# mp3guy/ElasticFusion

Measured on AMD Instinct MI355X. Metric: frames/s per GPU, 640x480 3-level ICP+fuse, higher is better.
Workload: dtype f32

## Files before the change

### elasticfusion_amd/csrc/ef_map_kernels.hip

```cpp
#include "ef_device.hpp"
#include <stdlib.h>
#include <mutex>
#include <hip/hip_ext.h>
#include "ef_map.hpp"
#include "ef_zkey.hpp"

using namespace ef;

namespace efm {

namespace {

inline int ceil_div(int a, int b) { return (a + b - 1) / b; }
constexpr int SURFEL_GRID = 1024;
constexpr int BLK = 256;
constexpr int CLEAN_GRID = 4096;
static_assert(CLEAN_ROW == BLK, "clean kernels run one element per thread");
static_assert(CLEAN_GRID % 8 == 0, "xcd_row");

__device__ __forceinline__ unsigned long long zkey(float z, uint32_t id) { return ((unsigned long long)depth_key(z) << 32) | id; }
__device__ __forceinline__ unsigned xcd_block() {
  const unsigned g = gridDim.x, x = blockIdx.x & 7u, slot = blockIdx.x >> 3;
  return x * (g >> 3) + (x < (g & 7u) ? x : (g & 7u)) + slot;
}
// ... 379 lines not shown
                                                        const unsigned* __restrict__ count_dev, float maxDepth, float confThreshold,
                                                        int time, int maxTime, int timeDelta, unsigned long long* zbuf,
                                                        unsigned* consumed_mark, unsigned consumed_value, const float4* __restrict__ rays) {
  if (consumed_mark && blockIdx.x == 0 && threadIdx.x == 0)
    __hip_atomic_store(consumed_mark, consumed_value, __ATOMIC_RELAXED, __HIP_MEMORY_SCOPE_SYSTEM);
  const rt34 T = rt34_load16(T16);
  const unsigned count = *count_dev;
  const unsigned sub = threadIdx.x % SPLAT_LANES;
  const unsigned stride = gridDim.x * blockDim.x / SPLAT_LANES;
  for (unsigned id = (blockIdx.x * blockDim.x + threadIdx.x) / SPLAT_LANES; id < count; id += stride) {
    const float4 pc = map.pos_conf[id];
    if (pc.w < confThreshold) continue;
    const float4 ct = map.col_time[id];
    const float4 nr = map.nrm_rad[id];
    const Sprite S = make_sprite(cam, T, pc, ct, nr, maxDepth, confThreshold, (float)time, (float)maxTime, (float)timeDelta);
    if (!S.ok) continue;
    const int px0 = max(0, (int)ceilf(S.u - S.hs - 0.5f)), px1 = min(cam.cols - 1, (int)ceilf(S.u + S.hs - 0.5f) - 1);
    const int py0 = max(0, (int)ceilf(S.v - S.hs - 0.5f)), py1 = min(cam.rows - 1, (int)ceilf(S.v + S.hs - 0.5f) - 1);
    const int hgt = py1 - py0 + 1, nfrag = (px1 - px0 + 1) * hgt;
    const float psn = dot(S.p, S.n);
    for (int f = (int)sub; f < nfrag; f += SPLAT_LANES) {
      const int fx = f / hgt, py = py0 + (f - fx * hgt), px = px0 + fx;
      const int zi = px * cam.rows + py;
      f3 l;
      if (LUT) { const float4 r = rays[zi]; l = f3{r.x, r.y, r.z}; }
      else l = pixel_ray(cam, px, py);
      float z;
      if (!sprite_fragment_ray(S.p, S.n, S.rad, psn, l, z)) continue;
      if (z != z) continue;
      unsigned long long* cell = &zbuf[zi];
      const unsigned long long key = zkey(z, id);
      atomicMin(cell, key);
    }
  }
}

__device__ __forceinline__ f3 fill_vertex_at(const uint16_t* __restrict__ d, const Cam& cam, int sx, int sy, int x, int y, float inv_fx,
                                             float inv_fy) {
  const float z = (float)d[clampi(sy, 0, cam.rows - 1) * cam.cols + clampi(sx, 0, cam.cols - 1)] / 1000.0f;
  return {((float)x - cam.cx) * z * inv_fx, ((float)y - cam.cy) * z * inv_fy, z};
}
__device__ __forceinline__ void fill_in_px(const Cam& cam, int x, int y, uchar4 si, float4 sv, float4 sn,
                                           const uint16_t* __restrict__ depth_filtered, const uint8_t* __restrict__ rgb3, bool passthrough,
                                           bool passthroughImage, FillMaps out) {
  const int pi = y * cam.cols + x;
  const float inv_fx = 1.0f / cam.fx, inv_fy = 1.0f / cam.fy;
  if (sv.z == 0 || passthrough) {
    const f3 v = fill_vertex_at(depth_filtered, cam, x, y, x, y, inv_fx, inv_fy);
    out.vertex[pi] = make_float4(v.x, v.y, v.z, 1.f);
  } else {
    out.vertex[pi] = sv;
  }
  if (sn.z == 0 || passthrough) {
    const f3 v = fill_vertex_at(depth_filtered, cam, x, y, x, y, inv_fx, inv_fy);
    const f3 vx = fill_vertex_at(depth_filtered, cam, x + 1, y, x + 1, y, inv_fx, inv_fy);
    const f3 vy = fill_vertex_at(depth_filtered, cam, x, y + 1, x, y + 1, inv_fx, inv_fy);
    const f3 nn = normalized(cross(vx - v, vy - v));
    out.normal[pi] = make_float4(nn.x, nn.y, nn.z, 1.f);
  } else {
    out.normal[pi] = sn;
  }
  if ((si.x == 0 && si.y == 0 && si.z == 0) || passthroughImage) {
    out.image[pi] = make_uchar4(rgb3[(size_t)pi * 3], rgb3[(size_t)pi * 3 + 1], rgb3[(size_t)pi * 3 + 2], 255);
  } else {
    out.image[pi] = si;
  }
}
__device__ __forceinline__ void dense_sample(const Cam& cam, int x, int y, uchar4 si, unsigned* counter) {
  if (counter && x % 20 == 10 && y % 20 == 10 && x / 20 < cam.cols / 20 && y / 20 < cam.rows / 20)
    if (si.x > 0 && si.y > 0 && si.z > 0) atomicAdd(counter, 1u);
}

template <bool FUSE_FILL>
__global__ void __launch_bounds__(BLK) k_surface_resolve(const Cam cam, const float* __restrict__ T16, SurfelSoA map, float maxDepth,
                                                          float confThreshold, int time, int maxTime, int timeDelta,
                                                          unsigned long long* zbuf, PredictMaps out, FillMaps fill,
                                                          const uint16_t* __restrict__ depth_filtered, const uint8_t* __restrict__ rgb3,
                                                          bool passthroughImage, unsigned* dense_counter, unsigned* nonempty_flag,
                                                          unsigned nonempty_value) {
  const int lane = threadIdx.x & 63, wave = threadIdx.x >> 6;
  const int px = blockIdx.x * 16 + (wave & 1) * 8 + (lane >> 3), py = blockIdx.y * 16 + (wave >> 1) * 8 + (lane & 7);
  if (px >= cam.cols || py >= cam.rows) return;
  const int pi = py * cam.cols + px, zi = px * cam.rows + py;
  const unsigned long long key = zbuf[zi];
  uchar4 im = make_uchar4(0, 0, 0, 0);
  float4 vt = make_float4(0, 0, 0, 0), nm = make_float4(0, 0, 0, 0);
  uint16_t tm = 0;
  if (key != ZBUF_EMPTY) {
    if (nonempty_flag) *nonempty_flag = nonempty_value;
    zbuf[zi] = ZBUF_EMPTY;
    const uint32_t id = (uint32_t)key;
    const rt34 T = rt34_load16(T16);
    const float4 pc = map.pos_conf[id], ct = map.col_time[id], nr = map.nrm_rad[id];
    const Sprite S = make_sprite(cam, T, pc, ct, nr, maxDepth, confThreshold, (float)time, (float)maxTime, (float)timeDelta);
    float z = 0.f;
    sprite_fragment(cam, S, px, py, z);
    const f3 col = decodeColor(ct.x);
    im = make_uchar4((uint8_t)roundf(col.x * 255.0f), (uint8_t)roundf(col.y * 255.0f), (uint8_t)roundf(col.z * 255.0f), 255);
    const float fcx = (float)px + 0.5f, fcy = (float)py + 0.5f;
    vt = make_float4((fcx - cam.cx) * z * (1.f / cam.fx), (fcy - cam.cy) * z * (1.f / cam.fy), z, pc.w);
    nm = make_float4(S.n.x, S.n.y, S.n.z, nr.w);
    tm = (uint16_t)(unsigned)ct.z;
  }
  out.image[pi] = im;
  out.vertex[pi] = vt;
  out.normal[pi] = nm;
  out.time[pi] = tm;
  if (FUSE_FILL) {
    fill_in_px(cam, px, py, im, vt, nm, depth_filtered, rgb3, false, passthroughImage, fill);
    dense_sample(cam, px, py, im, dense_counter);
  }
}
__global__ void __launch_bounds__(BLK) k_depth_resolve(int cols, int rows, unsigned long long* zbuf, float* __restrict__ depth) {
  const int pi = blockIdx.x * blockDim.x + threadIdx.x;
  if (pi >= cols * rows) return;
  const int py = pi / cols, px = pi - py * cols, zi = px * rows + py;
  const unsigned long long key = zbuf[zi];
  float z = 0.f;
  if (key != ZBUF_EMPTY) {
    zbuf[zi] = ZBUF_EMPTY;
    z = depth_of_key((uint32_t)(key >> 32));
  }
  depth[pi] = z;
}
__global__ void __launch_bounds__(BLK) k_fill_in(const Cam cam, PredictMaps pred, const uint16_t* __restrict__ depth_filtered,
                                                  const uint8_t* __restrict__ rgb3, bool passthrough, bool passthroughImage, FillMaps out) {
  const int pi = blockIdx.x * blockDim.x + threadIdx.x;
  if (pi >= cam.cols * cam.rows) return;
  const int py = pi / cam.cols, px = pi - py * cam.cols;
  fill_in_px(cam, px, py, pred.image[pi], pred.vertex[pi], pred.normal[pi], depth_filtered, rgb3, passthrough, passthroughImage, out);
}
__global__ void k_dense_count(const Cam cam, const uchar4* __restrict__ image, unsigned* counter) {
  const int dc = cam.cols / 20, dr = cam.rows / 20;
  const int i = blockIdx.x * blockDim.x + threadIdx.x;
  if (i >= dc * dr) return;
  const int b = i / dc, a = i - b * dc;
  const uchar4 t = image[(20 * b + 10) * cam.cols + (20 * a + 10)];
  if (t.x > 0 && t.y > 0 && t.z > 0) atomicAdd(counter, 1u);
}

struct FuseArgs {
  Cam cam;
  const float* pose16;
  int time;
  const uint8_t* rgb3;
  const float* dm;
  const float* dmf;
  IndexMaps im;
  float maxDepth;
  const float* weighting;
  KeyedIndex key;
  unsigned long long* zclear;
};
template <bool KEYED>
__global__ void __launch_bounds__(BLK) k_associate(const FuseArgs A, Candidates cand, uint32_t* winner, int colwalk) {
  const Cam cam = A.cam;
  const int qc = cam.cols / 2, qr = cam.rows / 2;
  const int q = (int)(xcd_block() * blockDim.x + threadIdx.x);
  if (KEYED && A.zclear)
    for (int i = q, P = cam.cols * cam.rows, step = (int)(gridDim.x * blockDim.x); i < P; i += step) A.zclear[i] = ZBUF_EMPTY;
  if (q >= qc * qr) return;
  const int qy = colwalk ? q % qr : q / qc, qx = colwalk ? q / qr : q - (q / qc) * qc;
  const int par = A.time % 2;
  const int i = 2 * qx + par, j = 2 * qy + par;
  const int r = qx * qr + qy;
  float4 c_col = make_float4(0, 0, 0, 0);
  if (i < cam.cols && j < cam.rows) {
    const float cx = cam.cx, cy = cam.cy;
    const float inv_fx = (float)(1.0 / (double)cam.fx), inv_fy = (float)(1.0 / (double)cam.fy);
    const DepthF DR{A.dm, cam.cols, cam.rows}, DF{A.dmf, cam.cols, cam.rows};
    const float x = pix_coord(i, cam.cols), y = pix_coord(j, cam.rows);
    const float ftime = (float)A.time;
    const f3 vPosLocal = getVertexF(DR, i, j, x, y, cx, cy, inv_fx, inv_fy);
    const bool sel = ((int)x % 2 == (int)ftime % 2 && (int)y % 2 == (int)ftime % 2);
    const bool nb = !(DR.at(i - 1, j) == 0 || DR.at(i, j - 1) == 0 || DR.at(i + 1, j) == 0 || DR.at(i, j + 1) == 0);
    const float zf_c = DF.at(i, j), zf_xf = DF.at(i + 1, j), zf_xb = DF.at(i - 1, j), zf_yf = DF.at(i, j + 1), zf_yb = DF.at(i, j - 1);
    const uint8_t* c = A.rgb3 + (size_t)(j * cam.cols + i) * 3;
    const uint8_t c0 = c[0], c1 = c[1], c2 = c[2];
    const float weighting = *A.weighting;
    uint32_t idx9[3][3];
    float4 vc9[3][3], nr9[3][3];
    uint2 key9[3][3];
#pragma unroll
    for (int a = 0; a < 3; ++a) {
      const int tx = clampi(i + a - 1, 0, cam.cols - 1);
#pragma unroll
      for (int b = 0; b < 3; ++b) {
        const int ty = clampi(j + b - 1, 0, cam.rows - 1);
        const int ti = im_texel(A.im, cam, tx, ty);
        if (KEYED) {
          key9[a][b] = reinterpret_cast<const uint2*>(A.key.keys)[ti];
        } else {
          idx9[a][b] = A.im.index[ti];
          vc9[a][b] = A.im.vert_conf[ti];
          nr9[a][b] = A.im.norm_rad[ti];
        }
      }
    }
    const rt34 pose = rt34_load16(A.pose16);
    if (sel && nb && vPosLocal.z > 0 && vPosLocal.z <= A.maxDepth) {
      const f3 vPos = xform(pose, vPosLocal);
      auto vtx = [&](float z, float xx, float yy) { return f3{(xx - cx) * z * inv_fx, (yy - cy) * z * inv_fy, z}; };
      const f3 vPosition_f = vtx(zf_c, x, y);
      const f3 col{(float)c0 / 255.0f, (float)c1 / 255.0f, (float)c2 / 255.0f};
      const f3 xf = vtx(zf_xf, x + 1, y), xb = vtx(zf_xb, x - 1, y), yf = vtx(zf_yf, x, y + 1), yb = vtx(zf_yb, x, y - 1);
      const f3 del_x = half_sum(xb, vPosition_f) - half_sum(xf, vPosition_f);
      const f3 del_y = half_sum(yb, vPosition_f) - half_sum(yf, vPosition_f);
      const f3 vNormLocal = normalized(cross(del_x, del_y));
      const f3 nW = mul(pose.R, vNormLocal);
      int counter = 0;
      uint32_t best = 0;
      float bestDist = 1000;
      const float xl = (x - cx) * inv_fx, yl = (y - cy) * inv_fy;
      const float lambda = sqrtf(xl * xl + yl * yl + 1);
      const f3 ray{xl, yl, 1};
      const float lenRay = sqrtf(dot(ray, ray));
      const float lenN = sqrtf(dot(vNormLocal, vNormLocal));
      const rt34 Tcw = rt34_load16(KEYED ? A.key.T_cw16_dev : A.pose16);
      if (KEYED) {
#pragma unroll
        for (int a = 0; a < 3; ++a)
#pragma unroll
          for (int b = 0; b < 3; ++b) {
            const uint32_t id = key9[a][b].x;
            float vcz = depth_of_key(key9[a][b].y);
            asm volatile("" : "+v"(vcz));
            const bool tap = (id & key9[a][b].y) != 0xFFFFFFFFu  && id > 0U && fabsf((vcz * lambda) - (vPosLocal.z * lambda)) < 0.05f;
            idx9[a][b] = tap ? id : 0U;
          }
#pragma unroll
        for (int a = 0; a < 3; ++a)
#pragma unroll
          for (int b = 0; b < 3; ++b) {
            vc9[a][b] = A.key.map.pos_conf[idx9[a][b]];
            nr9[a][b] = A.key.map.nrm_rad[idx9[a][b]];
          }
      }
#pragma unroll
      for (int a = 0; a < 4; ++a) {
        const int a3 = a == 0 ? 0 : (a == 3 ? 2 : 1);
#pragma unroll
        for (int b = 0; b < 4; ++b) {
          const int b3 = b == 0 ? 0 : (b == 3 ? 2 : 1);
          const uint32_t current = idx9[a3][b3];
          if (current > 0U) {
            const float4 vc = KEYED ? index_texel_vert_conf(Tcw, vc9[a3][b3]) : vc9[a3][b3];
            if (fabsf((vc.z * lambda) - (vPosLocal.z * lambda)) < 0.05f) {
              const f3 cr = cross(ray, f3{vc.x, vc.y, vc.z});
              const float dist = sqrtf(dot(cr, cr)) / lenRay;
              const float4 nr = KEYED ? index_texel_norm_rad(Tcw, nr9[a3][b3]) : nr9[a3][b3];
              const f3 nn{nr.x, nr.y, nr.z};
              const float cang = dot(nn, vNormLocal) / (sqrtf(dot(nn, nn)) * lenN);
              const bool angOk = (cang > 0.87758255f && cang <= 1.0f);
              if (dist < bestDist && (fabsf(nr.z) < 0.75f || angOk)) {
                counter++;
                bestDist = dist;
                best = current;
              }
            }
          }
        }
      }
      const float tag = counter > 0 ? -1.0f : -2.0f;
      cand.pos_conf[r] = make_float4(vPos.x, vPos.y, vPos.z, confidence(x, y, cx, cy, weighting));
      cand.nrm_rad[r] = make_float4(nW.x, nW.y, nW.z, getRadius(vPosition_f.z, vNormLocal.z, inv_fx, inv_fy));
      c_col = make_float4(encodeColor(col), 0.f, ftime, tag);
      cand.best[r] = best;
      if (counter > 0) atomicMin(&winner[best], (uint32_t)r);
    }
  }
  cand.col_time[r] = c_col;
}
__device__ __forceinline__ void merge_surfel(const Candidates& cand, int r, uint32_t id, const SurfelSoA& map, int time, float4& s, float4& sc) {
  const float4 ucol = cand.col_time[r];
  const float4 u = cand.pos_conf[r], un = cand.nrm_rad[r];
  float4 sn = map.nrm_rad[id];
  const float c_k = s.w, a = u.w, ftime = (float)time;
  if (un.w < (1.0f + 0.5f) * sn.w) {
    s.x = ((c_k * s.x) + (a * u.x)) / (c_k + a);
    s.y = ((c_k * s.y) + (a * u.y)) / (c_k + a);
    s.z = ((c_k * s.z) + (a * u.z)) / (c_k + a);
    s.w = c_k + a;
    const f3 oldCol = decodeColor(sc.x), newCol = decodeColor(ucol.x);
    const f3 avg{((c_k * oldCol.x) + (a * newCol.x)) / (c_k + a), ((c_k * oldCol.y) + (a * newCol.y)) / (c_k + a),
                 ((c_k * oldCol.z) + (a * newCol.z)) / (c_k + a)};
    sc.x = encodeColor(avg);
    sc.w = ftime;
    const float nx = ((c_k * sn.x) + (a * un.x)) / (c_k + a), ny = ((c_k * sn.y) + (a * un.y)) / (c_k + a),
                nz = ((c_k * sn.z) + (a * un.z)) / (c_k + a), nw = ((c_k * sn.w) + (a * un.w)) / (c_k + a);
    const f3 nn = normalized(f3{nx, ny, nz});
    sn = make_float4(nn.x, nn.y, nn.z, nw);
    map.pos_conf[id] = s;
    map.col_time[id] = sc;
    map.nrm_rad[id] = sn;
  } else {
    s.w = c_k + a;
    sc.w = ftime;
    map.pos_conf[id] = s;
    map.col_time[id] = sc;
  }
}
__global__ void __launch_bounds__(BLK) k_merge(Candidates cand, const uint32_t* __restrict__ winner, SurfelSoA map, int time) {
  const int r = blockIdx.x * blockDim.x + threadIdx.x;
  if (r >= cand.n) return;
  if (cand.col_time[r].w != -1.0f) return;
  const uint32_t id = cand.best[r];
  if (winner[id] != (uint32_t)r) return;
  float4 s = map.pos_conf[id], sc = map.col_time[id];
  merge_surfel(cand, r, id, map, time, s, sc);
}

struct CleanArgs {
  Cam cam;
  const float* T16;
  int time;
  IndexMaps im;
  float confThreshold;
  int timeDelta;
  KeyedIndex key;
};
struct Taps3 { int u[3]; int m[3]; };
__device__ __forceinline__ Taps3 dedupe_taps(float x, int hi) {
  int t[4];
#pragma unroll
  for (int a = 0; a < 4; ++a) t[a] = clampi((int)floorf(x + (-1.0f + 0.5f * a)), 0, hi);
  Taps3 r;
  r.u[0] = t[0];
  r.u[2] = t[3];
  r.u[1] = (t[1] != t[0] && t[1] != t[3]) ? t[1] : t[2];
  r.m[0] = 1 + (t[1] == t[0]) + (t[2] == t[0]) + (t[3] == t[0]);
  r.m[2] = (t[3] != t[0]) ? (1 + (t[0] == t[3]) + (t[1] == t[3]) + (t[2] == t[3])) : 0;
  r.m[1] = (r.u[1] != t[0] && r.u[1] != t[3]) ? ((t[1] == r.u[1]) + (t[2] == r.u[1])) : 0;
  return r;
}
template <bool KEYED>
__device__ __forceinline__ bool clean_test(const CleanArgs& A, const rt34& T, float4 pc, float4 ct, float4 nr) {
  const Cam& cam = A.cam;
  const float ftime = (float)A.time, ftd = (float)A.timeDelta;
  int test = 1;
  const f3 localPos = xform(T, f3{pc.x, pc.y, pc.z});
  const float x = ((cam.fx * localPos.x) / localPos.z) + cam.cx;
  const float y = ((cam.fy * localPos.y) / localPos.z) + cam.cy;
  const f3 localNorm = normalized(mul(T.R, f3{nr.x, nr.y, nr.z}));
  int cnt = 0, zCount = 0;
  const float tagTime = ct.w == -2 ? ftime : ct.w;
  const bool decided = tagTime == -1 || ((ftime - tagTime) > 20 && pc.w < A.confThreshold);
  if (!decided && ftime - ct.w < ftd && localPos.z > 0 && x > 0 && y > 0 && x < (float)cam.cols && y < (float)cam.rows) {
    const Taps3 tx = dedupe_taps(x, cam.cols - 1), ty = dedupe_taps(y, cam.rows - 1);
    uint32_t idx[9];
    float4 vcs[9], c2s[9];
    if (KEYED) {
      unsigned long long keys[9];
#pragma unroll
      for (int a = 0; a < 3; ++a)
#pragma unroll
        for (int b = 0; b < 3; ++b) keys[a * 3 + b] = A.key.keys[im_texel(A.im, cam, tx.u[a], ty.u[b])];
#pragma unroll
      for (int a = 0; a < 3; ++a)
#pragma unroll
        for (int b = 0; b < 3; ++b) {
          const unsigned long long key = keys[a * 3 + b];
          const uint32_t id = (uint32_t)key;
          const bool tap = tx.m[a] * ty.m[b] > 0 && key != ZBUF_EMPTY && id > 0U && depth_of_key((uint32_t)(key >> 32)) > localPos.z;
          idx[a * 3 + b] = tap ? id : 0U;
        }
#pragma unroll
      for (int k = 0; k < 9; ++k) {
        vcs[k] = A.key.map.pos_conf[idx[k]];
        c2s[k] = A.key.map.col_time[idx[k]];
      }
    } else {
#pragma unroll
      for (int a = 0; a < 3; ++a)
#pragma unroll
        for (int b = 0; b < 3; ++b) {
          const int ti = im_texel(A.im, cam, tx.u[a], ty.u[b]);
          idx[a * 3 + b] = A.im.index[ti];
          vcs[a * 3 + b] = A.im.vert_conf[ti];
          c2s[a * 3 + b] = A.im.color_time[ti];
        }
    }
    const bool steep = fabsf(localNorm.z) > 0.85f;
#pragma unroll
    for (int a = 0; a < 3; ++a)
#pragma unroll
      for (int b = 0; b < 3; ++b) {
        const int w = tx.m[a] * ty.m[b];
        const float4 vc = KEYED ? index_texel_vert_conf(T, vcs[a * 3 + b]) : vcs[a * 3 + b], c2 = c2s[a * 3 + b];
        if (w > 0 && idx[a * 3 + b] > 0U) {
          const float dx = vc.x - localPos.x, dy = vc.y - localPos.y;
          if (c2.z < ct.z && vc.w > A.confThreshold && vc.z > localPos.z && vc.z - localPos.z < 0.01f &&
              sqrtf(dx * dx + dy * dy) < nr.w * 1.4f)
            cnt += w;
          if (c2.w == ftime && vc.w > A.confThreshold && vc.z > localPos.z && vc.z - localPos.z > 0.01f && steep)
            zCount += w;
        }
      }
  }
  if (cnt > 8 || zCount > 4) test = 0;
  float lastTime = ct.w;
  if (lastTime == -2) lastTime = ftime;
  if (lastTime == -1 || ((ftime - lastTime) > 20 && pc.w < A.confThreshold)) test = 0;
  if (lastTime > 0 && ftime - lastTime > ftd) test = 1;
  return test != 0;
}
__device__ __forceinline__ bool load_element(const SurfelSoA& map, const Candidates& cand, unsigned count, unsigned e, float4& pc,
                                             float4& ct, float4& nr) {
  if (e < count) {
    pc = map.pos_conf[e]; ct = map.col_time[e]; nr = map.nrm_rad[e];
    return true;
  }
  const unsigned r = e - count;
  ct = cand.col_time[r];
  if (ct.w == 0.0f) return false;
  pc = cand.pos_conf[r]; nr = cand.nrm_rad[r];
  return true;
}
struct DeformArgs {
  const float* graph;
  int nodes;
  const float* depth;
  int isFern;
  float maxDepth;
};
// ... 263 lines not shown
    }
    base += tot;
    __syncthreads();
  }
}

}

static inline dim3 tgrid(int cols, int rows) { return dim3(ceil_div(cols, 64), ceil_div(rows, 4)); }

const float* bilateral_table() {
  static std::mutex mu;
  static float* tables[64] = {};
  int dev = 0;
  if (hipGetDevice(&dev) != hipSuccess || dev < 0 || dev >= 64) return nullptr;
  std::lock_guard<std::mutex> lk(mu);
  if (!tables[dev]) {
    float* p = nullptr;
    if (hipMalloc(&p, sizeof(float) * BIL_ROWS * BIL_COLS) != hipSuccess) return nullptr;
    hipLaunchKernelGGL(k_bilateral_table, dim3(ceil_div(BIL_ROWS * BIL_COLS, 256)), dim3(256), 0, (hipStream_t)0, p);
    if (hipDeviceSynchronize() != hipSuccess) { (void)hipFree(p); return nullptr; }
    tables[dev] = p;
  }
  return tables[dev];
}
bool filter_depth(const uint16_t* raw, int cols, int rows, float maxD, uint16_t* filtered, hipStream_t s) {
  const float* table = bilateral_table();
  if (!table) return false;
  hipLaunchKernelGGL(k_preprocess<false>, dim3(ceil_div(cols, PRE_TW), ceil_div(rows, PRE_TH)), dim3(64, 4), 0, s, raw, cols, rows, (unsigned)(maxD * 1000.0f), table,
                     filtered, (float*)nullptr, (float*)nullptr, (const uint8_t*)nullptr, (uint8_t*)nullptr, (uint8_t*)nullptr);
  return true;
}
void metricise_depth(const uint16_t* in, int cols, int rows, float maxD, float* out, hipStream_t s) {
  hipLaunchKernelGGL(k_metricise, dim3(ceil_div(cols * rows, 256)), dim3(256), 0, s, in, cols * rows, (unsigned)(maxD * 1000.0f), out);
}
bool preprocess_depth(const uint16_t* raw, int cols, int rows, float maxD, uint16_t* filtered, float* metric, float* metric_filtered,
                      hipStream_t s, unsigned extra_lds, const uint8_t* rgb3, uint8_t* next0, uint8_t* rgb_keep, const float* table) {
  if (!table) table = bilateral_table();
  if (!table) return false;
  constexpr unsigned STATIC_LDS = sizeof(float) * (BIL_ROWS * BIL_COLS + PRE_LH * PRE_LW);
  static_assert(STATIC_LDS < 65536u, "k_preprocess fits the default LDS limit");
  if (extra_lds > 65536u - STATIC_LDS) extra_lds = 65536u - STATIC_LDS;
  hipLaunchKernelGGL(k_preprocess<true>, dim3(ceil_div(cols, PRE_TW), ceil_div(rows, PRE_TH)), dim3(64, 4), extra_lds, s, raw, cols, rows, (unsigned)(maxD * 1000.0f), table,
                     filtered, metric, metric_filtered, rgb3, next0, rgb_keep);
  return true;
}
namespace {
__global__ void k_copy_map(SurfelSoA src, const unsigned* __restrict__ count_dev, SurfelSoA dst) {
  const unsigned n = *count_dev;
  for (unsigned i = blockIdx.x * blockDim.x + threadIdx.x; i < n; i += gridDim.x * blockDim.x) {
    dst.pos_conf[i] = src.pos_conf[i];
    dst.col_time[i] = src.col_time[i];
    dst.nrm_rad[i] = src.nrm_rad[i];
  }
}
}
void copy_map(SurfelSoA src, const unsigned* count_dev, SurfelSoA dst, hipStream_t s) {
  hipLaunchKernelGGL(k_copy_map, dim3(SURFEL_GRID), dim3(BLK), 0, s, src, count_dev, dst);
}
void aos_to_soa(const float* aos, uint32_t count, SurfelSoA soa, hipStream_t s) {
  if (count) hipLaunchKernelGGL(k_aos_to_soa, dim3(ceil_div((int)count, 256)), dim3(256), 0, s, (const float4*)aos, count, soa);
}
void soa_to_aos(SurfelSoA soa, uint32_t count, float* aos, hipStream_t s) {
  if (count) hipLaunchKernelGGL(k_soa_to_aos, dim3(ceil_div((int)count, 256)), dim3(256), 0, s, soa, count, (float4*)aos);
}

void seed_map(const Cam& cam, const uint8_t* rgb3, const float* dm, const float* dmf, int time, float maxDepth, SurfelSoA out,
              unsigned* count_dev, const CompactScratch& cs, hipStream_t s) {
  const int P = cam.cols * cam.rows;
  const int nch = ceil_div(P, CHUNK);
  SeedArgs A{cam, rgb3, dm, dmf, time, maxDepth};
  uint8_t* fr = cs.flags;
  uint8_t* ff = cs.flags + P;
  uint32_t* cr = cs.chunk_count;
  uint32_t* cf = cs.chunk_count + nch;
  uint32_t* orw = cs.chunk_offset;
  uint32_t* ofl = cs.chunk_offset + nch;
  (void)hipMemsetAsync(out.nrm_rad, 0, (size_t)P * sizeof(float4), s);
  hipLaunchKernelGGL(k_seed_flags, dim3(nch), dim3(BLK), 0, s, A, fr, ff, cr, cf);
  hipLaunchKernelGGL(k_scan_chunks, dim3(1), dim3(1024), 0, s, (const uint32_t*)cr, (const unsigned*)nullptr, (unsigned)P, orw, cs.totals);
  hipLaunchKernelGGL(k_scan_chunks, dim3(1), dim3(1024), 0, s, (const uint32_t*)cf, (const unsigned*)nullptr, (unsigned)P, ofl, cs.totals + 1);
  hipLaunchKernelGGL(k_seed_scatter, dim3(nch), dim3(BLK), 0, s, A, (const uint8_t*)fr, (const uint8_t*)ff, (const uint32_t*)orw,
                     (const uint32_t*)ofl, (const uint32_t*)cs.totals, out, count_dev);
}

void predict_indices(const Cam& cam, const float* T_cw16_dev, int time, SurfelSoA map, const unsigned* count_dev, float maxDepth,
                     int timeDelta, unsigned long long* zbuf, IndexMaps out, hipStream_t s, eft::KernelProbe* probe, const Candidates* merge_cand,
                     const uint32_t* merge_winner, bool resolve) {
  if (merge_cand) {
    hipLaunchKernelGGL(k_index_splat<true>, dim3(SURFEL_GRID), dim3(BLK), 0, s, cam, T_cw16_dev, time, map, count_dev, maxDepth, timeDelta, zbuf,
                       out.colmajor, *merge_cand, merge_winner);
    if (resolve) hipLaunchKernelGGL(k_index_resolve<true>, dim3(ceil_div(cam.cols * cam.rows, BLK)), dim3(BLK), 0, s, cam, T_cw16_dev, map, zbuf, out);
    return;
  }
  const bool sample = probe && probe->used < probe->capacity;
  hipEvent_t e0 = sample ? probe->start[probe->used] : nullptr, e1 = sample ? probe->stop[probe->used] : nullptr;
  if (sample) probe->used++;
  hipExtLaunchKernelGGL(k_index_splat<false>, dim3(SURFEL_GRID), dim3(BLK), 0, s, e0, e1, 0, cam, T_cw16_dev, time, map, count_dev, maxDepth, timeDelta,
                        zbuf, out.colmajor, Candidates{}, (const uint32_t*)nullptr);
  if (resolve) hipLaunchKernelGGL(k_index_resolve<true>, dim3(ceil_div(cam.cols * cam.rows, BLK)), dim3(BLK), 0, s, cam, T_cw16_dev, map, zbuf, out);
}
void resolve_indices(const Cam& cam, const float* T_cw16_dev, SurfelSoA map, const unsigned long long* zbuf, IndexMaps out, hipStream_t s) {
  hipLaunchKernelGGL(k_index_resolve<false>, dim3(ceil_div(cam.cols * cam.rows, BLK)), dim3(BLK), 0, s, cam, T_cw16_dev, map,
                     const_cast<unsigned long long*>(zbuf), out);
}

void combined_predict(const Cam& cam, const float* T_cw16_dev, SurfelSoA map, const unsigned* count_dev, float maxDepth,
                      float confThreshold, int time, int maxTime, int timeDelta, unsigned long long* zbuf, PredictMaps out, FillMaps fill,
                      const uint16_t* depth_filtered, const uint8_t* rgb3, bool passthroughImage, unsigned* dense_counter, hipStream_t s,
                      unsigned* nonempty_flag, unsigned nonempty_value, unsigned* consumed_mark, unsigned consumed_value, const float* rays4) {
  if (rays4)
    hipLaunchKernelGGL(k_surface_splat<true>, dim3(SPLAT_GRID), dim3(BLK), 0, s, cam, T_cw16_dev, map, count_dev, maxDepth, confThreshold,
                       time, maxTime, timeDelta, zbuf, consumed_mark, consumed_value, (const float4*)rays4);
  else
    hipLaunchKernelGGL(k_surface_splat<false>, dim3(SPLAT_GRID), dim3(BLK), 0, s, cam, T_cw16_dev, map, count_dev, maxDepth, confThreshold,
                       time, maxTime, timeDelta, zbuf, consumed_mark, consumed_value, (const float4*)nullptr);
  const dim3 g(ceil_div(cam.cols, 16), ceil_div(cam.rows, 16));
  if (fill.image)
    hipLaunchKernelGGL(k_surface_resolve<true>, g, dim3(BLK), 0, s, cam, T_cw16_dev, map, maxDepth, confThreshold, time, maxTime, timeDelta,
                       zbuf, out, fill, depth_filtered, rgb3, passthroughImage, dense_counter, nonempty_flag, nonempty_value);
  else
    hipLaunchKernelGGL(k_surface_resolve<false>, g, dim3(BLK), 0, s, cam, T_cw16_dev, map, maxDepth, confThreshold, time, maxTime, timeDelta,
                       zbuf, out, fill, depth_filtered, rgb3, passthroughImage, dense_counter, nonempty_flag, nonempty_value);
}
void synthesize_depth(const Cam& cam, const float* T_cw16_dev, SurfelSoA map, const unsigned* count_dev, float maxDepth, float confThreshold,
                      int time, int maxTime, int timeDelta, unsigned long long* zbuf, float* depth, hipStream_t s, const float* rays4) {
  if (rays4)
    hipLaunchKernelGGL(k_surface_splat<true>, dim3(SPLAT_GRID), dim3(BLK), 0, s, cam, T_cw16_dev, map, count_dev, maxDepth, confThreshold,
                       time, maxTime, timeDelta, zbuf, (unsigned*)nullptr, 0u, (const float4*)rays4);
  else
    hipLaunchKernelGGL(k_surface_splat<false>, dim3(SPLAT_GRID), dim3(BLK), 0, s, cam, T_cw16_dev, map, count_dev, maxDepth, confThreshold,
                       time, maxTime, timeDelta, zbuf, (unsigned*)nullptr, 0u, (const float4*)nullptr);
  const int n = cam.cols * cam.rows;
  hipLaunchKernelGGL(k_depth_resolve, dim3(ceil_div(n, BLK)), dim3(BLK), 0, s, cam.cols, cam.rows, zbuf, depth);
}
void build_ray_table(const Cam& cam, float* rays4, hipStream_t s) {
  hipLaunchKernelGGL(k_ray_table, dim3(ceil_div(cam.cols * cam.rows, BLK)), dim3(BLK), 0, s, cam, (float4*)rays4);
}
void fill_in(const Cam& cam, PredictMaps pred, const uint16_t* depth_filtered, const uint8_t* rgb3, bool passthrough, bool passthroughImage,
             FillMaps out, hipStream_t s) {
  hipLaunchKernelGGL(k_fill_in, dim3(ceil_div(cam.cols * cam.rows, BLK)), dim3(BLK), 0, s, cam, pred, depth_filtered, rgb3, passthrough,
                     passthroughImage, out);
}
void dense_count(const Cam& cam, const uchar4* image, unsigned* counter, hipStream_t s) {
  const int n = (cam.cols / 20) * (cam.rows / 20);
  hipLaunchKernelGGL(k_dense_count, dim3(ceil_div(n, 256)), dim3(256), 0, s, cam, image, counter);
}

void fuse(const Cam& cam, const float* pose_f16_dev, int time, const uint8_t* rgb3, const float* dm, const float* dmf, IndexMaps im,
          float maxDepth, const float* weighting_dev, SurfelSoA map, const unsigned* count_dev, Candidates cand, uint32_t* winner,
          hipStream_t s, bool defer_merge, const KeyedIndex* keyed, unsigned long long* zclear) {
  (void)count_dev;
  FuseArgs A{cam, pose_f16_dev, time, rgb3, dm, dmf, im, maxDepth, weighting_dev, keyed ? *keyed : KeyedIndex{}, zclear};
  if (keyed)
    hipLaunchKernelGGL(k_associate<true>, dim3(ceil_div(cand.n, BLK)), dim3(BLK), 0, s, A, cand, winner, im.colmajor ? 1 : 0);
  else
    hipLaunchKernelGGL(k_associate<false>, dim3(ceil_div(cand.n, BLK)), dim3(BLK), 0, s, A, cand, winner, im.colmajor ? 1 : 0);
  if (!defer_merge) hipLaunchKernelGGL(k_merge, dim3(ceil_div(cand.n, BLK)), dim3(BLK), 0, s, cand, (const uint32_t*)winner, map, time);
}

void clean(const Cam& cam, const float* T_cw16_dev, int time, IndexMaps im, float confThreshold, int timeDelta, SurfelSoA map,
           const unsigned* count_dev, Candidates cand, uint32_t* winner, SurfelSoA out, unsigned* count_out_dev, uint32_t capacity,
           CompactScratch& cs, int* overflow_flag, hipStream_t s, const Deformation* deform, const KeyedIndex* keyed,
           unsigned long long* zclear, float* T_keep16_dev) {
  CleanArgs A{cam, T_cw16_dev, time, im, confThreshold, timeDelta, keyed ? *keyed : KeyedIndex{}};
  const bool fold = cs.group_sum != nullptr;
  if (fold) cs.flip ^= 1;
  uint32_t* const gnow = fold ? cs.group_sum + (size_t)(cs.flip & 1) * cs.max_groups * CLEAN_GSTRIDE : nullptr;
  uint32_t* const gzero = fold ? cs.group_sum + (size_t)((cs.flip & 1) ^ 1) * cs.max_groups * CLEAN_GSTRIDE : nullptr;
  if (keyed)
    hipLaunchKernelGGL(k_clean_flags<true>, dim3(CLEAN_GRID), dim3(BLK), 0, s, A, map, count_dev, cand, winner, cs.flags,
                       cs.chunk_count, gnow, gzero, cs.max_groups);
  else
    hipLaunchKernelGGL(k_clean_flags<false>, dim3(CLEAN_GRID), dim3(BLK), 0, s, A, map, count_dev, cand, winner, cs.flags,
                       cs.chunk_count, gnow, gzero, cs.max_groups);
  if (deform && deform->nodes > 0) {
    const DeformArgs D{deform->graph_dev, deform->nodes, deform->depth_dev, deform->is_fern, deform->max_depth};
    hipLaunchKernelGGL(k_clean_deform, dim3(CLEAN_GRID), dim3(BLK), 0, s, A, D, map, count_dev, cand, (const uint8_t*)cs.flags);
  }
  if (!fold)
    hipLaunchKernelGGL(k_scan_chunks, dim3(1), dim3(1024), 0, s, (const uint32_t*)cs.chunk_count, (const unsigned*)count_dev, (unsigned)cand.n,
                       cs.chunk_offset, cs.totals, count_out_dev, capacity, overflow_flag, (unsigned)CLEAN_ROW);
  hipLaunchKernelGGL(k_clean_scatter, dim3(CLEAN_GRID), dim3(BLK), 0, s, map, count_dev, cand, (const uint8_t*)cs.flags,
                     (const uint32_t*)cs.chunk_offset, time, out, capacity, (const uint32_t*)gnow, (const uint32_t*)cs.chunk_count, cs.totals,
                     count_out_dev, overflow_flag, zclear, cam.cols * cam.rows, T_cw16_dev, T_keep16_dev);
}

void candidates_to_aos(Candidates cand, float* aos, unsigned* count_dev, const CompactScratch& cs, hipStream_t s) {
  const int nch = ceil_div(cand.n, CHUNK);
  hipLaunchKernelGGL(k_cand_flags, dim3(nch), dim3(BLK), 0, s, cand, cs.flags, cs.chunk_count);
  hipLaunchKernelGGL(k_scan_chunks, dim3(1), dim3(1024), 0, s, (const uint32_t*)cs.chunk_count, (const unsigned*)nullptr, (unsigned)cand.n,
                     cs.chunk_offset, count_dev);
  hipLaunchKernelGGL(k_cand_scatter, dim3(nch), dim3(BLK), 0, s, cand, (const uint8_t*)cs.flags, (const uint32_t*)cs.chunk_offset, (float4*)aos);
}

__global__ void k_sample_graph(SurfelSoA map, const unsigned* __restrict__ count_dev, int stride, int max_nodes, float4* __restrict__ out,
                               unsigned* __restrict__ n_out) {
  const int i = blockIdx.x * blockDim.x + threadIdx.x;
  const unsigned count = *count_dev;
  const unsigned n = count == 0 ? 0u : (count - 1u) / (unsigned)stride + 1u;
  if (i == 0) *n_out = n < (unsigned)max_nodes ? n : (unsigned)max_nodes;
  if (i >= max_nodes || (unsigned)i >= n) return;
  const float4 p = map.pos_conf[(size_t)i * stride];
  const float4 c = map.col_time[(size_t)i * stride];
  out[i] = make_float4(p.x, p.y, p.z, c.z);
}
void sample_graph(SurfelSoA map, const unsigned* count_dev, int stride, int max_nodes, float* out4, unsigned* n_out, hipStream_t s) {
  hipLaunchKernelGGL(k_sample_graph, dim3(ceil_div(max_nodes, 256)), dim3(256), 0, s, map, count_dev, stride, max_nodes, (float4*)out4, n_out);
}

#include "ef_render.inc"
#include "ef_labels.inc"
#include "ef_query.inc"
#include "ef_register.inc"

}
```

Baseline: 2130.

## Split fuse association neighbourhood search across four lanes with DPP reduction

k_associate now assigns four threads to each candidate pixel. Each lane evaluates a contiguous slice of the 3x3 index-map neighbourhood (ceil(9/4) slots), instead of one thread walking a 4x4 loop that revisits the centre and edge taps. Lanes reduce their best (distance, id) with DPP quad permutes, and only lane 0 does the pose transform, colour encode and candidate writes. The aim is more memory-level parallelism and fewer live registers per thread for the gather-heavy search. The cost is a grid four times larger, per-pixel setup (depth loads, normal estimation) repeated in every lane, and lanes idling on padded slots.

Result: faster. 2166, median of 6 (+1.7%).

```diff
diff --git a/elasticfusion_amd/csrc/ef_map_kernels.hip b/elasticfusion_amd/csrc/ef_map_kernels.hip
--- a/elasticfusion_amd/csrc/ef_map_kernels.hip
+++ b/elasticfusion_amd/csrc/ef_map_kernels.hip
@@ -555,14 +555,35 @@
   KeyedIndex key;
   unsigned long long* zclear;
 };
+constexpr int ASSOC_LANES = 4;
+constexpr int ASSOC_SLOTS = (9 + ASSOC_LANES - 1) / ASSOC_LANES;
+static_assert(ASSOC_LANES == 1 || ASSOC_LANES == 2 || ASSOC_LANES == 4 || ASSOC_LANES == 8, "a wavefront holds whole pixels; the combine knows offsets 1, 2, 4");
+template <int OFF>
+__device__ __forceinline__ uint32_t assoc_lane_down(uint32_t v) {
+  static_assert(OFF == 1 || OFF == 2 || OFF == 4, "");
+  constexpr int ctrl = OFF == 1 ? 0xF5  : OFF == 2 ? 0xEE  : 0x104 ;
+  return (uint32_t)__builtin_amdgcn_update_dpp(0, (int)v, ctrl, 0xF, 0xF, true);
+}
+template <int OFF>
+__device__ __forceinline__ void assoc_combine(float& bestDist, uint32_t& best) {
+  const float d = __uint_as_float(assoc_lane_down<OFF>(__float_as_uint(bestDist)));
+  const uint32_t id = assoc_lane_down<OFF>(best);
+  if (d < bestDist) {
+    bestDist = d;
+    best = id;
+  }
+}
 template <bool KEYED>
 __global__ void __launch_bounds__(BLK) k_associate(const FuseArgs A, Candidates cand, uint32_t* winner, int colwalk) {
   const Cam cam = A.cam;
   const int qc = cam.cols / 2, qr = cam.rows / 2;
-  const int q = (int)(xcd_block() * blockDim.x + threadIdx.x);
+  const int t = (int)(xcd_block() * blockDim.x + threadIdx.x);
   if (KEYED && A.zclear)
-    for (int i = q, P = cam.cols * cam.rows, step = (int)(gridDim.x * blockDim.x); i < P; i += step) A.zclear[i] = ZBUF_EMPTY;
+    for (int i = t, P = cam.cols * cam.rows, step = (int)(gridDim.x * blockDim.x); i < P; i += step) A.zclear[i] = ZBUF_EMPTY;
+  const int q = t / ASSOC_LANES, sub = t % ASSOC_LANES;
   if (q >= qc * qr) return;
+  const int seg_len = 9 / ASSOC_LANES + (sub < 9 % ASSOC_LANES ? 1 : 0);
+  const int seg_first = sub * (9 / ASSOC_LANES) + (sub < 9 % ASSOC_LANES ? sub : 9 % ASSOC_LANES);
   const int qy = colwalk ? q % qr : q / qc, qx = colwalk ? q / qr : q - (q / qc) * qc;
   const int par = A.time % 2;
   const int i = 2 * qx + par, j = 2 * qy + par;
@@ -581,37 +602,32 @@
     const uint8_t* c = A.rgb3 + (size_t)(j * cam.cols + i) * 3;
     const uint8_t c0 = c[0], c1 = c[1], c2 = c[2];
     const float weighting = *A.weighting;
-    uint32_t idx9[3][3];
-    float4 vc9[3][3], nr9[3][3];
-    uint2 key9[3][3];
-#pragma unroll
-    for (int a = 0; a < 3; ++a) {
-      const int tx = clampi(i + a - 1, 0, cam.cols - 1);
-#pragma unroll
-      for (int b = 0; b < 3; ++b) {
-        const int ty = clampi(j + b - 1, 0, cam.rows - 1);
-        const int ti = im_texel(A.im, cam, tx, ty);
-        if (KEYED) {
-          key9[a][b] = reinterpret_cast<const uint2*>(A.key.keys)[ti];
-        } else {
-          idx9[a][b] = A.im.index[ti];
-          vc9[a][b] = A.im.vert_conf[ti];
-          nr9[a][b] = A.im.norm_rad[ti];
-        }
+    uint32_t idxs[ASSOC_SLOTS];
+    float4 vcs[ASSOC_SLOTS], nrs[ASSOC_SLOTS];
+    uint2 keys[ASSOC_SLOTS];
+#pragma unroll
+    for (int m = 0; m < ASSOC_SLOTS; ++m) {
+      const int k = m < seg_len ? seg_first + m : 8;
+      const int a3 = (k >= 3) + (k >= 6), b3 = k - 3 * a3;
+      const int tx = clampi(i + a3 - 1, 0, cam.cols - 1), ty = clampi(j + b3 - 1, 0, cam.rows - 1);
+      const int ti = im_texel(A.im, cam, tx, ty);
+      if (KEYED) {
+        keys[m] = reinterpret_cast<const uint2*>(A.key.keys)[ti];
+      } else {
+        const uint32_t id = A.im.index[ti];
+        idxs[m] = m < seg_len ? id : 0U;
+        vcs[m] = A.im.vert_conf[ti];
+        nrs[m] = A.im.norm_rad[ti];
       }
     }
     const rt34 pose = rt34_load16(A.pose16);
     if (sel && nb && vPosLocal.z > 0 && vPosLocal.z <= A.maxDepth) {
-      const f3 vPos = xform(pose, vPosLocal);
       auto vtx = [&](float z, float xx, float yy) { return f3{(xx - cx) * z * inv_fx, (yy - cy) * z * inv_fy, z}; };
       const f3 vPosition_f = vtx(zf_c, x, y);
-      const f3 col{(float)c0 / 255.0f, (float)c1 / 255.0f, (float)c2 / 255.0f};
       const f3 xf = vtx(zf_xf, x + 1, y), xb = vtx(zf_xb, x - 1, y), yf = vtx(zf_yf, x, y + 1), yb = vtx(zf_yb, x, y - 1);
       const f3 del_x = half_sum(xb, vPosition_f) - half_sum(xf, vPosition_f);
       const f3 del_y = half_sum(yb, vPosition_f) - half_sum(yf, vPosition_f);
       const f3 vNormLocal = normalized(cross(del_x, del_y));
-      const f3 nW = mul(pose.R, vNormLocal);
-      int counter = 0;
       uint32_t best = 0;
       float bestDist = 1000;
       const float xl = (x - cx) * inv_fx, yl = (y - cy) * inv_fy;
@@ -622,57 +638,56 @@
       const rt34 Tcw = rt34_load16(KEYED ? A.key.T_cw16_dev : A.pose16);
       if (KEYED) {
 #pragma unroll
-        for (int a = 0; a < 3; ++a)
-#pragma unroll
-          for (int b = 0; b < 3; ++b) {
-            const uint32_t id = key9[a][b].x;
-            float vcz = depth_of_key(key9[a][b].y);
-            asm volatile("" : "+v"(vcz));
-            const bool tap = (id & key9[a][b].y) != 0xFFFFFFFFu  && id > 0U && fabsf((vcz * lambda) - (vPosLocal.z * lambda)) < 0.05f;
-            idx9[a][b] = tap ? id : 0U;
-          }
-#pragma unroll
-        for (int a = 0; a < 3; ++a)
-#pragma unroll
-          for (int b = 0; b < 3; ++b) {
-            vc9[a][b] = A.key.map.pos_conf[idx9[a][b]];
-            nr9[a][b] = A.key.map.nrm_rad[idx9[a][b]];
-          }
+        for (int m = 0; m < ASSOC_SLOTS; ++m) {
+          const uint32_t id = keys[m].x;
+          float vcz = depth_of_key(keys[m].y);
+          asm volatile("" : "+v"(vcz));
+          const bool tap = m < seg_len && (id & keys[m].y) != 0xFFFFFFFFu  && id > 0U && fabsf((vcz * lambda) - (vPosLocal.z * lambda)) < 0.05f;
+          idxs[m] = tap ? id : 0U;
+        }
+#pragma unroll
+        for (int m = 0; m < ASSOC_SLOTS; ++m) {
+          vcs[m] = A.key.map.pos_conf[idxs[m]];
+          nrs[m] = A.key.map.nrm_rad[idxs[m]];
+        }
       }
 #pragma unroll
-      for (int a = 0; a < 4; ++a) {
-        const int a3 = a == 0 ? 0 : (a == 3 ? 2 : 1);
-#pragma unroll
-        for (int b = 0; b < 4; ++b) {
-          const int b3 = b == 0 ? 0 : (b == 3 ? 2 : 1);
-          const uint32_t current = idx9[a3][b3];
-          if (current > 0U) {
-            const float4 vc = KEYED ? index_texel_vert_conf(Tcw, vc9[a3][b3]) : vc9[a3][b3];
-            if (fabsf((vc.z * lambda) - (vPosLocal.z * lambda)) < 0.05f) {
-              const f3 cr = cross(ray, f3{vc.x, vc.y, vc.z});
-              const float dist = sqrtf(dot(cr, cr)) / lenRay;
-              const float4 nr = KEYED ? index_texel_norm_rad(Tcw, nr9[a3][b3]) : nr9[a3][b3];
-              const f3 nn{nr.x, nr.y, nr.z};
-              const float cang = dot(nn, vNormLocal) / (sqrtf(dot(nn, nn)) * lenN);
-              const bool angOk = (cang > 0.87758255f && cang <= 1.0f);
-              if (dist < bestDist && (fabsf(nr.z) < 0.75f || angOk)) {
-                counter++;
-                bestDist = dist;
-                best = current;
-              }
+      for (int m = 0; m < ASSOC_SLOTS; ++m) {
+        const uint32_t current = idxs[m];
+        if (current > 0U) {
+          const float4 vc = KEYED ? index_texel_vert_conf(Tcw, vcs[m]) : vcs[m];
+          if (fabsf((vc.z * lambda) - (vPosLocal.z * lambda)) < 0.05f) {
+            const f3 cr = cross(ray, f3{vc.x, vc.y, vc.z});
+            const float dist = sqrtf(dot(cr, cr)) / lenRay;
+            const float4 nr = KEYED ? index_texel_norm_rad(Tcw, nrs[m]) : nrs[m];
+            const f3 nn{nr.x, nr.y, nr.z};
+            const float cang = dot(nn, vNormLocal) / (sqrtf(dot(nn, nn)) * lenN);
+            const bool angOk = (cang > 0.87758255f && cang <= 1.0f);
+            if (dist < bestDist && (fabsf(nr.z) < 0.75f || angOk)) {
+              bestDist = dist;
+              best = current;
             }
           }
         }
       }
-      const float tag = counter > 0 ? -1.0f : -2.0f;
-      cand.pos_conf[r] = make_float4(vPos.x, vPos.y, vPos.z, confidence(x, y, cx, cy, weighting));
-      cand.nrm_rad[r] = make_float4(nW.x, nW.y, nW.z, getRadius(vPosition_f.z, vNormLocal.z, inv_fx, inv_fy));
-      c_col = make_float4(encodeColor(col), 0.f, ftime, tag);
-      cand.best[r] = best;
-      if (counter > 0) atomicMin(&winner[best], (uint32_t)r);
-    }
-  }
-  cand.col_time[r] = c_col;
+      if (ASSOC_LANES > 1) assoc_combine<1>(bestDist, best);
+      if (ASSOC_LANES > 2) assoc_combine<2>(bestDist, best);
+      if (ASSOC_LANES > 4) assoc_combine<4>(bestDist, best);
+      if (sub == 0) {
+        const bool found = bestDist < 1000;
+        const f3 vPos = xform(pose, vPosLocal);
+        const f3 nW = mul(pose.R, vNormLocal);
+        const f3 col{(float)c0 / 255.0f, (float)c1 / 255.0f, (float)c2 / 255.0f};
+        const float tag = found ? -1.0f : -2.0f;
+        cand.pos_conf[r] = make_float4(vPos.x, vPos.y, vPos.z, confidence(x, y, cx, cy, weighting));
+        cand.nrm_rad[r] = make_float4(nW.x, nW.y, nW.z, getRadius(vPosition_f.z, vNormLocal.z, inv_fx, inv_fy));
+        c_col = make_float4(encodeColor(col), 0.f, ftime, tag);
+        cand.best[r] = best;
+        if (found) atomicMin(&winner[best], (uint32_t)r);
+      }
+    }
+  }
+  if (sub == 0) cand.col_time[r] = c_col;
 }
 __device__ __forceinline__ void merge_surfel(const Candidates& cand, int r, uint32_t id, const SurfelSoA& map, int time, float4& s, float4& sc) {
   const float4 ucol = cand.col_time[r];
@@ -1242,10 +1257,11 @@
           hipStream_t s, bool defer_merge, const KeyedIndex* keyed, unsigned long long* zclear) {
   (void)count_dev;
   FuseArgs A{cam, pose_f16_dev, time, rgb3, dm, dmf, im, maxDepth, weighting_dev, keyed ? *keyed : KeyedIndex{}, zclear};
+  const int groups = ceil_div(cand.n * ASSOC_LANES, BLK);
   if (keyed)
-    hipLaunchKernelGGL(k_associate<true>, dim3(ceil_div(cand.n, BLK)), dim3(BLK), 0, s, A, cand, winner, im.colmajor ? 1 : 0);
+    hipLaunchKernelGGL(k_associate<true>, dim3(groups), dim3(BLK), 0, s, A, cand, winner, im.colmajor ? 1 : 0);
   else
-    hipLaunchKernelGGL(k_associate<false>, dim3(ceil_div(cand.n, BLK)), dim3(BLK), 0, s, A, cand, winner, im.colmajor ? 1 : 0);
+    hipLaunchKernelGGL(k_associate<false>, dim3(groups), dim3(BLK), 0, s, A, cand, winner, im.colmajor ? 1 : 0);
   if (!defer_merge) hipLaunchKernelGGL(k_merge, dim3(ceil_div(cand.n, BLK)), dim3(BLK), 0, s, cand, (const uint32_t*)winner, map, time);
 }
 
```
